# lhn0323/BEVFUSION-3D_object_detection

Hardware: AMD Instinct MI355X
Metric: nuScenes frames/sec (6-cam+LiDAR BEVFusion fwd+bwd) (higher is better)
Workload: dtype bf16; 1 GPU; full: BEVFusion camera+LiDAR (ResNet-50, LSS 6x256x704, hard voxelize 40k pts, sparse encoder, ConvFuser, SECOND/SECONDFPN, TransFusion head + Hungarian targets + focal/L1/gaussian-focal losses) fwd + bwd + clip + AdamW, bf16 autocast, fp32 index paths; global_batch=4, points_per_frame=40000, parallelism=independent frames per rank, execution=eager launches on 2 HIP queues (camera / BEV chain, LiDAR branch), view_transform_conv_dtype=bf16, head_fp32_conv=three bf16 products per multiply, fp32 accumulation (2^-16 relative per product), dense_weight_gradients=one grouped launch per tile shape at the end of the backward pass, backward_pass_thread=caller, trainable_params=37361053

## Files before the change

### bevfusion-3d_object_detection_amd/_lib.py

```python
import ctypes
import os

import torch

_HERE = os.path.dirname(os.path.abspath(__file__))
LIB_PATH = os.path.join(_HERE, "csrc", "libbevfusion_hip.so")

_c_int = ctypes.c_int
_c_vp = ctypes.c_void_p
_c_sz = ctypes.c_size_t

SIGNATURES = {
    "bfhip_abi_version": (_c_int, []),
    "bfhip_last_error": (ctypes.c_char_p, []),
    "bfhip_profile_enable": (None, [_c_int]),
    "bfhip_profile_read": (_c_int, [_c_int, _c_vp, _c_vp, _c_int]),
    "bfhip_bev_pool_fwd": (_c_int, [_c_vp] * 5 + [_c_int] * 7 + [_c_vp, _c_vp]),
    "bfhip_bev_pool_bwd": (_c_int, [_c_vp] * 5 + [_c_int] * 8 + [_c_vp, _c_vp]),
    "bfhip_dynamic_voxelize": (_c_int, [_c_vp, _c_vp, _c_int, _c_int, _c_vp, _c_vp, _c_vp]),
    "bfhip_hard_voxelize_workspace_bytes": (_c_sz, [_c_int, _c_int, _c_int]),
    "bfhip_hard_voxelize": (_c_int, [_c_vp, _c_int, _c_int, _c_vp, _c_vp, _c_vp, _c_vp, _c_vp,
                                     _c_int, _c_int, _c_vp, _c_sz, _c_vp, _c_vp]),
    "bfhip_bev_plan_workspace_bytes": (_c_sz, [ctypes.c_longlong, ctypes.c_longlong]),
    "bfhip_bev_plan": (_c_int, [_c_vp] * 7 + [_c_int] * 4 + [_c_vp] * 3 + [_c_vp] * 11 + [_c_int, _c_vp, _c_sz, _c_vp]),
# ... 22 lines not shown
    "bfhip_sparse_to_bev": (_c_int, [_c_vp, _c_vp] + [_c_int] * 6 + [_c_vp, _c_vp]),
    "bfhip_bev_to_sparse": (_c_int, [_c_vp, _c_vp] + [_c_int] * 6 + [_c_vp, _c_vp]),
    "bfhip_dynamic_scatter_workspace_bytes": (_c_sz, [_c_int]),
    "bfhip_dynamic_scatter_fwd": (_c_int, [_c_vp, _c_vp, _c_int, _c_int, _c_int] + [_c_vp] * 5 + [_c_vp, _c_sz, _c_vp]),
    "bfhip_dynamic_scatter_bwd_workspace_bytes": (_c_sz, [_c_int, _c_int]),
    "bfhip_dynamic_scatter_bwd": (_c_int, [_c_vp] * 6 + [_c_int] * 4 + [_c_vp, _c_sz, _c_vp]),
    "bfhip_voxel_mean": (_c_int, [_c_vp, _c_vp, _c_int, _c_int, _c_int, _c_vp, _c_vp]),
    "bfhip_voxel_compact_mean": (_c_int, [_c_vp] * 4 + [_c_int] * 5 + [_c_vp] * 4),
    "bfhip_depth_lift_bwd_workspace_bytes": (_c_sz, []),
    "bfhip_depth_lift_bwd": (_c_int, [_c_vp, _c_vp, ctypes.c_longlong, _c_vp, _c_vp, _c_sz, _c_vp]),
    "bfhip_rasterise_depth_workspace_bytes": (_c_sz, [_c_int] * 3),
    "bfhip_rasterise_depth": (_c_int, [_c_vp, _c_int, _c_int] + [_c_vp] * 4 + [_c_int] * 3 + [_c_vp, _c_vp] + [_c_int] * 3 +
                              [_c_vp, _c_vp, _c_sz, _c_vp]),
    "bfhip_depth_histogram": (_c_int, [_c_vp] + [_c_int] * 6 + [_c_vp, _c_vp, _c_vp, _c_vp]),
    "bfhip_bn1d_workspace_bytes": (_c_sz, [_c_int, _c_int]),
    "bfhip_bn1d_fwd": (_c_int, [_c_vp] * 4 + [_c_int, _c_int, ctypes.c_float, ctypes.c_float, _c_int] + [_c_vp] * 5 +
                       [_c_vp, _c_sz, _c_vp]),
    "bfhip_bn1d_bwd": (_c_int, [_c_vp] * 5 + [_c_int] * 3 + [_c_vp] * 4 + [_c_vp, _c_sz, _c_vp]),
    "bfhip_sparse_to_bev_nhwc": (_c_int, [_c_vp, _c_vp] + [_c_int] * 7 + [_c_vp, _c_vp]),
    "bfhip_bev_nhwc_to_sparse": (_c_int, [_c_vp, ctypes.c_longlong, ctypes.c_longlong, ctypes.c_longlong, _c_int, _c_vp, _c_int,
                                          _c_int, _c_int, _c_vp, _c_vp]),
    "bfhip_bn2d_supported": (_c_int, [ctypes.c_longlong, _c_int, _c_int]),
    "bfhip_bn2d_workspace_bytes": (_c_sz, [ctypes.c_longlong, _c_int, _c_int]),
    "bfhip_colsum": (_c_int, [_c_vp, ctypes.c_longlong, _c_int, _c_int, _c_vp, _c_vp, _c_sz, _c_vp]),
    "bfhip_bn2d_fwd": (_c_int, [_c_vp] * 4 + [ctypes.c_longlong, _c_int, _c_int, ctypes.c_float, ctypes.c_float, _c_int] +
                       [_c_vp] * 5 + [_c_vp, _c_sz, _c_vp]),
    "bfhip_bn2d_bwd": (_c_int, [_c_vp] * 5 + [ctypes.c_longlong, _c_int, _c_int, _c_int] + [_c_vp] * 4 + [_c_vp, _c_sz, _c_vp]),
    "bfhip_xty_workspace_bytes": (_c_sz, [ctypes.c_longlong, _c_int, _c_int]),
    "bfhip_xty": (_c_int, [_c_vp, _c_vp, ctypes.c_longlong, _c_int, _c_int, _c_int, _c_vp, _c_vp, _c_sz, _c_vp]),
    "bfhip_attn_max_queries": (_c_int, []),
    "bfhip_attn_workspace_bytes": (_c_sz, [_c_int] * 4),
    "bfhip_attn_fwd": (_c_int, [_c_vp] * 3 + [_c_int] * 4 + [ctypes.c_float, ctypes.c_float, ctypes.c_ulonglong, _c_vp, _c_vp,
                                                             _c_vp, _c_vp, _c_sz, _c_vp]),
    "bfhip_attn_bwd": (_c_int, [_c_vp] * 6 + [_c_int] * 4 + [ctypes.c_float, ctypes.c_float, ctypes.c_ulonglong] + [_c_vp] * 4 +
                       [_c_vp, _c_sz, _c_vp]),
    "bfhip_attn_dropout_mask": (_c_int, [_c_int] * 4 + [ctypes.c_float, ctypes.c_ulonglong, _c_vp, _c_vp, _c_vp]),
    "bfhip_upsample2x_nhwc": (_c_int, [_c_vp, _c_vp] + [_c_int] * 6 + [_c_vp]),
    "bfhip_maxpool3x3s2_fwd": (_c_int, [_c_vp] + [_c_int] * 4 + [_c_vp, _c_vp, _c_vp]),
    "bfhip_maxpool3x3s2_bwd": (_c_int, [_c_vp, _c_vp] + [_c_int] * 4 + [_c_vp, _c_vp]),
    "bfhip_circle_nms": (_c_int, [_c_vp, _c_int, ctypes.c_float, _c_int, _c_vp, _c_vp, _c_vp]),
    "bfhip_rotate_nms_workspace_bytes": (_c_sz, [_c_int, _c_int]),
    "bfhip_rotate_nms": (_c_int, [_c_vp, _c_vp, _c_int, ctypes.c_float, _c_int, _c_int, _c_vp, _c_vp, _c_vp, _c_sz, _c_vp]),
    "bfhip_decode_boxes": (_c_int, [_c_vp] * 5 + [_c_int] * 4 + [_c_vp, _c_vp, _c_vp]),
    "bfhip_assign_cost": (_c_int, [_c_vp, _c_int, _c_vp, _c_int, _c_int, _c_int, _c_vp, _c_int, _c_vp, _c_vp] + [_c_int] * 3 +
                          [_c_vp] * 4),
    "bfhip_hungarian": (_c_int, [_c_vp, _c_vp, _c_int, _c_int, _c_int, _c_vp, _c_vp, _c_vp]),
# ... 181 lines not shown
```

### bevfusion-3d_object_detection_amd/csrc/bn2d.hip

```cpp
#include <algorithm>
#include <map>
#include <mutex>

#include "common.h"

namespace bfhip {
namespace {

typedef unsigned short bf16_t;

template <typename T> struct Vec;
template <> struct Vec<float> {
  static constexpr int V = 4;
  static __device__ __forceinline__ void load(const float *p, float *o) {
    float4 v = *(const float4 *)p;
    o[0] = v.x; o[1] = v.y; o[2] = v.z; o[3] = v.w;
  }
  static __device__ __forceinline__ void store(float *p, const float *o) { *(float4 *)p = make_float4(o[0], o[1], o[2], o[3]); }
};
template <> struct Vec<bf16_t> {
  static constexpr int V = 8;
  static __device__ __forceinline__ void load(const bf16_t *p, float *o) {
    uint4 v = *(const uint4 *)p;
    const unsigned w[4] = {v.x, v.y, v.z, v.w};
#pragma unroll
    for (int i = 0; i < 4; ++i) {
      o[2 * i] = __uint_as_float(w[i] << 16);
      o[2 * i + 1] = __uint_as_float(w[i] & 0xffff0000u);
    }
  }
  static __device__ __forceinline__ unsigned rne(float f) {
    unsigned u = __float_as_uint(f);
    if ((u & 0x7fffffffu) > 0x7f800000u) return (u >> 16) | 0x40u;
    return (u + 0x7fffu + ((u >> 16) & 1u)) >> 16;
  }
  static __device__ __forceinline__ void store(bf16_t *p, const float *o) {
    uint4 v;
    v.x = rne(o[0]) | (rne(o[1]) << 16);
    v.y = rne(o[2]) | (rne(o[3]) << 16);
    v.z = rne(o[4]) | (rne(o[5]) << 16);
    v.w = rne(o[6]) | (rne(o[7]) << 16);
    *(uint4 *)p = v;
  }
};
// ... 71 lines not shown
    st_agent(&cnt[1 + g], 0);
    s_flag = __hip_atomic_fetch_add(&cnt[0], 1, __ATOMIC_RELAXED, __HIP_MEMORY_SCOPE_AGENT) == tr.ng - 1;
  }
  __syncthreads();
  if (!s_flag) return;
  if (t == 0) st_agent(&cnt[0], 0);
  if (own) {
    double s = 0.0, s2 = 0.0;
    for (int g2 = 0; g2 < tr.ng; ++g2) {
      s += ld_agent(&tr.gp[((size_t)g2 * 2 + 0) * C + c]);
      s2 += ld_agent(&tr.gp[((size_t)g2 * 2 + 1) * C + c]);
    }
    fin(c, s, s2);
  }
}

struct FwdFin {
  long long M;
  const int *m_dev;
  int C;
  float eps, momentum;
  const float *gamma, *beta;
  float *stats, *running_mean, *running_var;
  __device__ __forceinline__ void operator()(int c, double s, double s2) const {
    long long Mv = M;
    if (m_dev) { long long mv = *m_dev; Mv = mv < 1 ? 1 : (mv < M ? mv : M); }
    double mean = s / (double)Mv;
    double var = s2 / (double)Mv - mean * mean;
    if (var < 0.0) var = 0.0;
    float invstd = (float)(1.0 / sqrt(var + (double)eps));
    float a = gamma[c] * invstd;
    stats[c] = (float)mean;
    stats[C + c] = invstd;
    stats[2 * C + c] = a;
    stats[3 * C + c] = beta[c] - (float)mean * a;
    if (running_mean) {
      double unbiased = Mv > 1 ? var * (double)Mv / (double)(Mv - 1) : var;
      running_mean[c] = (float)((1.0 - momentum) * running_mean[c] + momentum * mean);
      running_var[c] = (float)((1.0 - momentum) * running_var[c] + momentum * unbiased);
    }
  }
};

struct BwdFin {
  long long M;
  const int *m_dev;
  int C;
  const float *stats;
  float *dgb, *coef;
  __device__ __forceinline__ void operator()(int c, double s, double s2) const {
    long long Mv = M;
    if (m_dev) { long long mv = *m_dev; Mv = mv < 1 ? 1 : (mv < M ? mv : M); }
    const float mean = stats[c], invstd = stats[C + c], a = stats[2 * C + c];
    const float dbeta = (float)s, dgamma = (float)(s2 * (double)invstd);
    dgb[c] = dgamma;
    dgb[C + c] = dbeta;
    const float invM = (float)(1.0 / (double)Mv);
    const float c2 = -a * invstd * dgamma * invM;
    coef[c] = a;
    coef[C + c] = c2;
    coef[2 * C + c] = -a * dbeta * invM - c2 * mean;
  }
};

struct SumFin {
  int C;
  float *out;
  __device__ __forceinline__ void operator()(int c, double s, double) const { out[c] = (float)s; }
};

template <typename T>
__global__ __launch_bounds__(256) void bn2d_stats_kernel(const T *__restrict__ x, long long M, int C, Map mp,
                                                         float *__restrict__ partial, Tree tr, FwdFin fin) {
  constexpr int V = Vec<T>::V;
  __shared__ float sm[2 * 256 * V];
  const int t = threadIdx.x, cv = blockIdx.y * mp.Lb + t % mp.Lb, rl = t / mp.Lb;
  const bool live = rl < mp.R && cv * V < C;
  float s0[V], s1[V];
#pragma unroll
  for (int j = 0; j < V; ++j) { s0[j] = 0.f; s1[j] = 0.f; }
  if (live) {
    const long long r0 = (long long)blockIdx.x * mp.rpb, r1 = r0 + mp.rpb < M ? r0 + mp.rpb : M;
    const T *p = x + (size_t)cv * V;
    long long r = r0 + rl;
    for (; r + 3LL * mp.R < r1; r += 4LL * mp.R) {
      float v[4][V];
#pragma unroll
      for (int u = 0; u < 4; ++u) Vec<T>::load(p + (size_t)(r + (long long)u * mp.R) * C, v[u]);
#pragma unroll
      for (int u = 0; u < 4; ++u)
#pragma unroll
        for (int j = 0; j < V; ++j) { s0[j] += v[u][j]; s1[j] += v[u][j] * v[u][j]; }
    }
    for (; r < r1; r += mp.R) {
      float v[V];
      Vec<T>::load(p + (size_t)r * C, v);
#pragma unroll
      for (int j = 0; j < V; ++j) { s0[j] += v[j]; s1[j] += v[j] * v[j]; }
    }
  }
  combine_rows<V>(s0, s1, mp.Lb, mp.R, C, partial, sm);
  finish_in_last_block(partial, tr, C, blockIdx.y * mp.Lb * V, mp.Lb * V, fin);
}

constexpr int kFinLanes = 64, kFinThreads = 8 * kFinLanes;
__device__ __forceinline__ void reduce_partials8(const float *__restrict__ partial, int nblk, int C, int c, bool ok,
                                                 double &s, double &s2) {
  __shared__ double sm[2][kFinThreads];
  const int t = threadIdx.x, kl = t >> 3;
  double a = 0.0, b = 0.0;
  if (ok) {
    for (int k0 = kl; k0 < nblk; k0 += 16 * kFinLanes) {
      float v0[16], v1[16];
#pragma unroll
      for (int u = 0; u < 16; ++u) {
        const int k = k0 + u * kFinLanes, kc = k < nblk ? k : nblk - 1;
        v0[u] = partial[((size_t)kc * 2 + 0) * C + c];
        v1[u] = partial[((size_t)kc * 2 + 1) * C + c];
      }
#pragma unroll
      for (int u = 0; u < 16; ++u)
        if (k0 + u * kFinLanes < nblk) { a += (double)v0[u]; b += (double)v1[u]; }
    }
  }
  sm[0][t] = a;
  sm[1][t] = b;
  __syncthreads();
  double x = 0.0, y = 0.0;
  if (t < 64) {
    const int ch = t & 7, g = t >> 3;
#pragma unroll
    for (int j = 0; j < 8; ++j) { x += sm[0][(g * 8 + j) * 8 + ch]; y += sm[1][(g * 8 + j) * 8 + ch]; }
  }
  __syncthreads();
  if (t < 64) { sm[0][t] = x; sm[1][t] = y; }
  __syncthreads();
  s = 0.0; s2 = 0.0;
  if (t < 8)
#pragma unroll
    for (int g = 0; g < 8; ++g) { s += sm[0][g * 8 + t]; s2 += sm[1][g * 8 + t]; }
}

template <typename Fin>
__global__ __launch_bounds__(kFinThreads) void bn2d_finalize_kernel(const float *__restrict__ partial, int nblk, Fin fin) {
  const int c = blockIdx.x * 8 + (threadIdx.x & 7);
  double s, s2;
  reduce_partials8(partial, nblk, fin.C, c, c < fin.C, s, s2);
  if (threadIdx.x >= 8 || c >= fin.C) return;
  fin(c, s, s2);
}

template <typename T, bool RES, bool RELU>
__global__ __launch_bounds__(256) void bn2d_apply_kernel(const T *__restrict__ x, const T *__restrict__ res,
                                                         const float *__restrict__ stats, long long M, int C, Map mp,
                                                         T *__restrict__ y, unsigned char *__restrict__ relu_mask) {
  constexpr int V = Vec<T>::V;
  const int t = threadIdx.x, cv = blockIdx.y * mp.Lb + t % mp.Lb, rl = t / mp.Lb;
  const bool live = rl < mp.R && cv * V < C;
  if (!live) return;
  float a[V], b[V];
#pragma unroll
  for (int j = 0; j < V; ++j) { a[j] = stats[2 * C + cv * V + j]; b[j] = stats[3 * C + cv * V + j]; }
  const long long r0 = (long long)blockIdx.x * mp.rpb, r1 = r0 + mp.rpb < M ? r0 + mp.rpb : M;
  const size_t col = (size_t)cv * V;
  long long r = r0 + rl;
  for (; r + mp.R < r1; r += 2LL * mp.R) {
    float v[2][V], q[2][V];
#pragma unroll
    for (int u = 0; u < 2; ++u) {
      Vec<T>::load(x + (size_t)(r + (long long)u * mp.R) * C + col, v[u]);
      if (RES) Vec<T>::load(res + (size_t)(r + (long long)u * mp.R) * C + col, q[u]);
    }
// ... 8 lines not shown
        v[u][j] = (RELU && !(o > 0.f)) ? 0.f : o;
      }
      Vec<T>::store(y + (size_t)(r + (long long)u * mp.R) * C + col, v[u]);
      if (V == 8 && relu_mask) relu_mask[(size_t)(r + (long long)u * mp.R) * (C >> 3) + cv] = (unsigned char)bits;
    }
  }
  for (; r < r1; r += mp.R) {
    float v[V], q[V];
    Vec<T>::load(x + (size_t)r * C + col, v);
    if (RES) Vec<T>::load(res + (size_t)r * C + col, q);
    unsigned bits = 0;
#pragma unroll
    for (int j = 0; j < V; ++j) {
      float o = v[j] * a[j] + b[j];
      if (RES) o += q[j];
      if (o > 0.f) bits |= 1u << j;
      v[j] = (RELU && !(o > 0.f)) ? 0.f : o;
    }
    Vec<T>::store(y + (size_t)r * C + col, v);
    if (V == 8 && relu_mask) relu_mask[(size_t)r * (C >> 3) + cv] = (unsigned char)bits;
  }
}

template <typename T, int MASK>
__device__ __forceinline__ void masked_grad(float *g, const float *xv, const float *yv, const float *a, const float *b) {
  constexpr int V = Vec<T>::V;
  const unsigned bits = MASK == 3 ? __float_as_uint(yv[0]) : 0u;
#pragma unroll
  for (int j = 0; j < V; ++j) {
    if (MASK == 1 && !(xv[j] * a[j] + b[j] > 0.f)) g[j] = 0.f;
    if (MASK == 2 && !(yv[j] > 0.f)) g[j] = 0.f;
    if (MASK == 3 && !((bits >> j) & 1u)) g[j] = 0.f;
  }
}

template <typename T, int MASK>
__global__ __launch_bounds__(256) void bn2d_bwd_reduce_kernel(const T *__restrict__ dy, const T *__restrict__ x,
                                                              const T *__restrict__ y,
                                                              const float *__restrict__ stats, long long M, int C,
                                                              Map mp, float *__restrict__ partial, Tree tr, BwdFin fin) {
  constexpr int V = Vec<T>::V;
  __shared__ float sm[2 * 256 * V];
  const int t = threadIdx.x, cv = blockIdx.y * mp.Lb + t % mp.Lb, rl = t / mp.Lb;
  const bool live = rl < mp.R && cv * V < C;
  float s0[V], s1[V];
#pragma unroll
  for (int j = 0; j < V; ++j) { s0[j] = 0.f; s1[j] = 0.f; }
  if (live) {
    float mean[V], a[V], b[V];
#pragma unroll
    for (int j = 0; j < V; ++j) {
      mean[j] = stats[cv * V + j];
      a[j] = stats[2 * C + cv * V + j];
      b[j] = stats[3 * C + cv * V + j];
    }
    const long long r0 = (long long)blockIdx.x * mp.rpb, r1 = r0 + mp.rpb < M ? r0 + mp.rpb : M;
// ... 67 lines not shown
#pragma unroll
    for (int u = 0; u < 2; ++u) {
      size_t off = (size_t)(r + (long long)u * mp.R) * C + col;
      masked_grad<T, MASK>(g[u], xv[u], yv[u], a, b);
      if (DRES) Vec<T>::store(dres + off, g[u]);
#pragma unroll
      for (int j = 0; j < V; ++j) xv[u][j] = c1[j] * g[u][j] + c2[j] * xv[u][j] + c3[j];
      Vec<T>::store(dx + off, xv[u]);
    }
  }
  for (; r < r1; r += mp.R) {
    float g[V], xv[V], yv[V];
    size_t off = (size_t)r * C + col;
    Vec<T>::load(dy + off, g);
    Vec<T>::load(x + off, xv);
    if (MASK == 2) Vec<T>::load(y + off, yv);
    if (MASK == 3) yv[0] = __uint_as_float(((const unsigned char *)y)[(size_t)r * (C >> 3) + cv]);
    masked_grad<T, MASK>(g, xv, yv, a, b);
    if (DRES) Vec<T>::store(dres + off, g);
#pragma unroll
    for (int j = 0; j < V; ++j) xv[j] = c1[j] * g[j] + c2[j] * xv[j] + c3[j];
    Vec<T>::store(dx + off, xv);
  }
}

inline int elem_size(int dtype) { return dtype == 1 ? 2 : 4; }

inline bool shape_ok(long long M, int C, int dtype) {
  const int V = 16 / elem_size(dtype);
  return M > 0 && C >= V && C % V == 0 && C <= 65536;
}

inline Map make_map(long long M, int C, int dtype, dim3 *grid) {
  const int es = elem_size(dtype), V = 16 / es, L = C / V;
  Map mp;
  mp.Lb = L < 32 ? L : 32;
  mp.R = 256 / mp.Lb;
  const int CT = (L + mp.Lb - 1) / mp.Lb;
  long long S = 1024;
  S = std::min(S, (M + 4LL * mp.R - 1) / (4LL * mp.R));
  S = std::min(S, (long long)std::max(1, 2048 / CT));
  S = std::min(S, std::max(1LL, M * es / 128));
  S = std::max(S, 1LL);
  long long rpb = ((M + S - 1) / S + mp.R - 1) / mp.R * mp.R;
  S = (M + rpb - 1) / rpb;
  mp.rpb = (int)rpb;
  *grid = dim3((unsigned)S, (unsigned)CT);
  return mp;
}

template <typename T>
int run_fwd(const void *x, const void *res, const float *stats, long long M, int C, Map mp, dim3 grid, int relu, void *y,
            hipStream_t s, unsigned char *relu_mask = nullptr) {
#define BFHIP_BN2D_APPLY(RES, RELU)                                                                             \
  hipLaunchKernelGGL((bn2d_apply_kernel<T, RES, RELU>), grid, dim3(256), 0, s, (const T *)x, (const T *)res, \
                     stats, M, C, mp, (T *)y, (RES && RELU) ? relu_mask : (unsigned char *)nullptr)
  if (res) { if (relu) BFHIP_BN2D_APPLY(true, true); else BFHIP_BN2D_APPLY(true, false); }
  else { if (relu) BFHIP_BN2D_APPLY(false, true); else BFHIP_BN2D_APPLY(false, false); }
#undef BFHIP_BN2D_APPLY
  return 0;
}

template <typename T, int MASK>
void run_bwd(const void *dy, const void *x, const void *y, const float *stats, long long M, int C, Map mp, dim3 grid,
             float *partial, float *coef, Tree tr, BwdFin fin, void *dx, void *dres, hipStream_t s) {
  hipLaunchKernelGGL((bn2d_bwd_reduce_kernel<T, MASK>), grid, dim3(256), 0, s, (const T *)dy, (const T *)x,
                     (const T *)y, stats, M, C, mp, partial, tr, fin);
  if (!tr.cnt) hipLaunchKernelGGL(bn2d_finalize_kernel<BwdFin>, dim3(ceil_div(C, 8)), dim3(kFinThreads), 0, s, partial, tr.nblk, fin);
  if (dres)
    hipLaunchKernelGGL((bn2d_bwd_apply_kernel<T, MASK, true>), grid, dim3(256), 0, s, (const T *)dy, (const T *)x,
                       (const T *)y, stats, coef, M, C, mp, (T *)dx, (T *)dres);
  else
    hipLaunchKernelGGL((bn2d_bwd_apply_kernel<T, MASK, false>), grid, dim3(256), 0, s, (const T *)dy,
                       (const T *)x, (const T *)y, stats, coef, M, C, mp, (T *)dx, (T *)nullptr);
}

constexpr int kSlabInts = 16384;
constexpr int kSlabs = 32;

inline bool fold_enabled() {
  static const bool on = [] { const char *e = env_str("BFHIP_BN2D_FOLD"); return e && e[0] == '1'; }();
  return on;
}

int *arrival_counters(hipStream_t stream) {
  static std::mutex mu;
  static std::map<int, int *> pool;
  static std::map<std::pair<int, hipStream_t>, int> slot;
  static std::map<int, int> used;
  int dev = 0;
  if (hipGetDevice(&dev) != hipSuccess) return nullptr;
  std::lock_guard<std::mutex> lock(mu);
  auto it = pool.find(dev);
  if (it == pool.end()) {
    int *p = nullptr;
    const size_t bytes = (size_t)kSlabs * kSlabInts * sizeof(int);
    if (hipMalloc((void **)&p, bytes) != hipSuccess || hipMemset(p, 0, bytes) != hipSuccess) {
// ... 25 lines not shown
  pl->ng = (pl->nblk + kGroup - 1) / kGroup;
  size_t off = 0;
  pl->partial = (float *)((char *)workspace + off); off += align_up((size_t)pl->nblk * 2 * C * sizeof(float), 256);
  pl->coef = (float *)((char *)workspace + off); off += align_up((size_t)3 * C * sizeof(float), 256);
  pl->gp = (double *)((char *)workspace + off); off += align_up((size_t)pl->ng * 2 * C * sizeof(double), 256);
  return off;
}

}
}

using namespace bfhip;

BFHIP_EXPORT int bfhip_bn2d_supported(long long M, int C, int dtype) {
  return (dtype == 0 || dtype == 1) && shape_ok(M, C, dtype) ? 1 : 0;
}

BFHIP_EXPORT size_t bfhip_bn2d_workspace_bytes(long long M, int C, int dtype) {
  if (!bfhip_bn2d_supported(M, C, dtype)) return 0;
  Plan pl;
  return plan_bytes(M, C, dtype, &pl, nullptr);
}

BFHIP_EXPORT int bfhip_colsum(const void *x, long long M, int C, int dtype, float *out, void *workspace, size_t workspace_bytes,
                              void *stream_) {
  hipStream_t s = (hipStream_t)stream_;
  BFHIP_REQUIRE(bfhip_bn2d_supported(M, C, dtype), "colsum: unsupported shape M=%lld C=%d dtype=%d", M, C, dtype);
  BFHIP_REQUIRE(x && out && ((uintptr_t)x % 16) == 0, "colsum: null or misaligned pointer");
  if (!workspace || workspace_bytes < bfhip_bn2d_workspace_bytes(M, C, dtype)) { set_error("colsum: workspace too small"); return BFHIP_E_WORKSPACE; }
  Plan pl;
  plan_bytes(M, C, dtype, &pl, workspace);
  Tree tr{nullptr, pl.gp, pl.nblk, pl.ng};
  FwdFin none{};
  if (dtype == 1)
    hipLaunchKernelGGL(bn2d_stats_kernel<bf16_t>, pl.grid, dim3(256), 0, s, (const bf16_t *)x, M, C, pl.mp, pl.partial, tr, none);
  else
    hipLaunchKernelGGL(bn2d_stats_kernel<float>, pl.grid, dim3(256), 0, s, (const float *)x, M, C, pl.mp, pl.partial, tr, none);
  hipLaunchKernelGGL(bn2d_finalize_kernel<SumFin>, dim3(ceil_div(C, 8)), dim3(kFinThreads), 0, s, pl.partial, pl.nblk, SumFin{C, out});
  return check_launch("colsum");
}

BFHIP_EXPORT int bfhip_bn2d_fwd(const void *x, const void *residual, const float *gamma, const float *beta,
                                long long M, int C, int dtype, float eps, float momentum, int relu,
                                float *running_mean, float *running_var, float *stats, void *y, const int32_t *m_dev,
                                void *workspace, size_t workspace_bytes, void *stream_) {
  hipStream_t s = (hipStream_t)stream_;
  BFHIP_REQUIRE(bfhip_bn2d_supported(M, C, dtype), "bn2d_fwd: unsupported shape M=%lld C=%d dtype=%d", M, C, dtype);
  BFHIP_REQUIRE(x && gamma && beta && stats && y, "bn2d_fwd: null pointer");
  BFHIP_REQUIRE(((uintptr_t)x % 16) == 0 && ((uintptr_t)y % 16) == 0 && ((uintptr_t)residual % 16) == 0,
                "bn2d_fwd: tensors must be 16-byte aligned");
  if (!workspace || workspace_bytes < bfhip_bn2d_workspace_bytes(M, C, dtype)) { set_error("bn2d_fwd: workspace too small"); return BFHIP_E_WORKSPACE; }
  Plan pl;
  plan_bytes(M, C, dtype, &pl, workspace);
  int *cnt = fold_enabled() ? arrival_counters(s) : nullptr;
  if (!cnt && fold_enabled()) return BFHIP_E_LAUNCH;
  BFHIP_REQUIRE((long long)pl.grid.y * (1 + pl.ng) <= kSlabInts, "bn2d_fwd: too many column tiles");
  Tree tr{cnt, pl.gp, pl.nblk, pl.ng};
  FwdFin fin{M, m_dev, C, eps, momentum, gamma, beta, stats, running_mean, running_var};
  ProfScope ps;
  prof_begin(BFHIP_OP_BN2D_FWD, s, &ps);
  if (dtype == 1)
    hipLaunchKernelGGL(bn2d_stats_kernel<bf16_t>, pl.grid, dim3(256), 0, s, (const bf16_t *)x, M, C, pl.mp, pl.partial, tr, fin);
  else
    hipLaunchKernelGGL(bn2d_stats_kernel<float>, pl.grid, dim3(256), 0, s, (const float *)x, M, C, pl.mp, pl.partial, tr, fin);
  if (!cnt) hipLaunchKernelGGL(bn2d_finalize_kernel<FwdFin>, dim3(ceil_div(C, 8)), dim3(kFinThreads), 0, s, pl.partial, pl.nblk, fin);
  if (dtype == 1) run_fwd<bf16_t>(x, residual, stats, M, C, pl.mp, pl.grid, relu, y, s);
  else run_fwd<float>(x, residual, stats, M, C, pl.mp, pl.grid, relu, y, s);
  prof_end(&ps);
  return check_launch("bn2d_fwd");
}

static int bn2d_fwd_partials_impl(const void *x, const void *residual, const float *gamma, const float *beta, long long M, int C,
                                  int dtype, float eps, float momentum, int relu, float *running_mean, float *running_var,
                                  float *stats, void *y, const float *partial, int nblk, const int32_t *m_dev,
                                  unsigned char *relu_mask, void *stream_) {
  hipStream_t s = (hipStream_t)stream_;
  BFHIP_REQUIRE(!relu_mask || (dtype == 1 && relu && residual), "bn2d_fwd_partials: a ReLU bit mask needs bf16 + residual + ReLU");
  BFHIP_REQUIRE(bfhip_bn2d_supported(M, C, dtype), "bn2d_fwd_partials: unsupported shape M=%lld C=%d dtype=%d", M, C, dtype);
  BFHIP_REQUIRE(x && gamma && beta && stats && y && partial && nblk > 0, "bn2d_fwd_partials: null pointer");
  BFHIP_REQUIRE(((uintptr_t)x % 16) == 0 && ((uintptr_t)y % 16) == 0 && ((uintptr_t)residual % 16) == 0,
                "bn2d_fwd_partials: tensors must be 16-byte aligned");
  dim3 grid;
  Map mp = make_map(M, C, dtype, &grid);
  FwdFin fin{M, m_dev, C, eps, momentum, gamma, beta, stats, running_mean, running_var};
  ProfScope ps;
  prof_begin(BFHIP_OP_BN2D_FWD, s, &ps);
  hipLaunchKernelGGL(bn2d_finalize_kernel<FwdFin>, dim3(ceil_div(C, 8)), dim3(kFinThreads), 0, s, partial, nblk, fin);
  if (dtype == 1) run_fwd<bf16_t>(x, residual, stats, M, C, mp, grid, relu, y, s, relu_mask);
  else run_fwd<float>(x, residual, stats, M, C, mp, grid, relu, y, s);
  prof_end(&ps);
  return check_launch("bn2d_fwd_partials");
}

BFHIP_EXPORT int bfhip_bn2d_fwd_partials(const void *x, const void *residual, const float *gamma, const float *beta,
                                         long long M, int C, int dtype, float eps, float momentum, int relu,
                                         float *running_mean, float *running_var, float *stats, void *y,
                                         const float *partial, int nblk, const int32_t *m_dev, void *stream_) {
  return bn2d_fwd_partials_impl(x, residual, gamma, beta, M, C, dtype, eps, momentum, relu, running_mean, running_var, stats, y,
                                partial, nblk, m_dev, nullptr, stream_);
}

BFHIP_EXPORT int bfhip_bn2d_fwd_partials_mask(const void *x, const void *residual, const float *gamma, const float *beta,
                                              long long M, int C, int dtype, float eps, float momentum, int relu,
                                              float *running_mean, float *running_var, float *stats, void *y,
                                              const float *partial, int nblk, const int32_t *m_dev, unsigned char *relu_mask,
                                              void *stream_) {
  BFHIP_REQUIRE(relu_mask, "bn2d_fwd_partials_mask: null mask");
  return bn2d_fwd_partials_impl(x, residual, gamma, beta, M, C, dtype, eps, momentum, relu, running_mean, running_var, stats, y,
                                partial, nblk, m_dev, relu_mask, stream_);
}

static int bn2d_bwd_impl(const void *dy, const void *x, const void *y, const unsigned char *relu_mask, const float *stats,
                         const float *gamma, long long M, int C, int dtype, int relu, void *dx, void *dres, float *dgb,
                         const int32_t *m_dev, void *workspace, size_t workspace_bytes, void *stream_) {
  hipStream_t s = (hipStream_t)stream_;
  BFHIP_REQUIRE(!relu_mask || (dtype == 1 && relu), "bn2d_bwd: a ReLU bit mask needs bf16 + ReLU");
  if (relu_mask) y = relu_mask;
  BFHIP_REQUIRE(bfhip_bn2d_supported(M, C, dtype), "bn2d_bwd: unsupported shape M=%lld C=%d dtype=%d", M, C, dtype);
  BFHIP_REQUIRE(dy && x && stats && gamma && dx && dgb, "bn2d_bwd: null pointer");
  BFHIP_REQUIRE(((uintptr_t)dy % 16) == 0 && ((uintptr_t)x % 16) == 0 && ((uintptr_t)dx % 16) == 0 &&
                    ((uintptr_t)y % 16) == 0 && ((uintptr_t)dres % 16) == 0, "bn2d_bwd: tensors must be 16-byte aligned");
  if (!workspace || workspace_bytes < bfhip_bn2d_workspace_bytes(M, C, dtype)) { set_error("bn2d_bwd: workspace too small"); return BFHIP_E_WORKSPACE; }
  Plan pl;
  plan_bytes(M, C, dtype, &pl, workspace);
  int *cnt = fold_enabled() ? arrival_counters(s) : nullptr;
  if (!cnt && fold_enabled()) return BFHIP_E_LAUNCH;
  BFHIP_REQUIRE((long long)pl.grid.y * (1 + pl.ng) <= kSlabInts, "bn2d_bwd: too many column tiles");
  Tree tr{cnt, pl.gp, pl.nblk, pl.ng};
  BwdFin fin{M, m_dev, C, stats, dgb, pl.coef};
  const int mask = !relu ? 0 : (relu_mask ? 3 : (y ? 2 : 1));
  ProfScope ps;
  prof_begin(BFHIP_OP_BN2D_BWD, s, &ps);
#define BFHIP_BN2D_BWD(T, MASK) run_bwd<T, MASK>(dy, x, y, stats, M, C, pl.mp, pl.grid, pl.partial, pl.coef, tr, fin, dx, dres, s)
  if (dtype == 1) {
    if (mask == 0) BFHIP_BN2D_BWD(bf16_t, 0);
    else if (mask == 1) BFHIP_BN2D_BWD(bf16_t, 1);
    else if (mask == 3) BFHIP_BN2D_BWD(bf16_t, 3);
    else BFHIP_BN2D_BWD(bf16_t, 2);
  } else {
    if (mask == 0) BFHIP_BN2D_BWD(float, 0);
    else if (mask == 1) BFHIP_BN2D_BWD(float, 1);
    else BFHIP_BN2D_BWD(float, 2);
  }
#undef BFHIP_BN2D_BWD
  prof_end(&ps);
  return check_launch("bn2d_bwd");
}

BFHIP_EXPORT int bfhip_bn2d_bwd(const void *dy, const void *x, const void *y, const float *stats, const float *gamma,
                                long long M, int C, int dtype, int relu, void *dx, void *dres, float *dgb,
                                const int32_t *m_dev, void *workspace, size_t workspace_bytes, void *stream_) {
  return bn2d_bwd_impl(dy, x, y, nullptr, stats, gamma, M, C, dtype, relu, dx, dres, dgb, m_dev, workspace, workspace_bytes, stream_);
}

BFHIP_EXPORT int bfhip_bn2d_bwd_mask(const void *dy, const void *x, const unsigned char *relu_mask, const float *stats,
                                     const float *gamma, long long M, int C, int dtype, void *dx, void *dres, float *dgb,
// ... 6 lines not shown
```

### include/bevfusion_hip.h

```cpp
#ifndef BEVFUSION_HIP_H_
#define BEVFUSION_HIP_H_

#include <stddef.h>
#include <stdint.h>

#ifdef __cplusplus
extern "C" {
#endif

#define BFHIP_OK 0
#define BFHIP_E_INVALID (-1)
#define BFHIP_E_WORKSPACE (-2)
#define BFHIP_E_LAUNCH (-3)

#define BFHIP_REDUCE_SUM 0
#define BFHIP_REDUCE_MEAN 1
#define BFHIP_REDUCE_MAX 2

#define BFHIP_OP_BEV_POOL_FWD 0
#define BFHIP_OP_BEV_POOL_BWD 1
#define BFHIP_OP_HARD_VOXELIZE 2
#define BFHIP_OP_DYNAMIC_VOXELIZE 3
#define BFHIP_OP_LIFT_SPLAT_FWD 4
#define BFHIP_OP_LIFT_SPLAT_BWD 5
// ... 125 lines not shown
                             int dtype, const int32_t *indices, int N, int C, int Z, float *grad_feats, void *stream);

size_t bfhip_depth_lift_bwd_workspace_bytes(void);
int bfhip_depth_lift_bwd(const void *dy, const void *d, long long M, float *out, void *workspace, size_t workspace_bytes, void *stream);
size_t bfhip_rasterise_depth_workspace_bytes(int ncam, int iH, int iW);
int bfhip_rasterise_depth(const float *points, int n, int f, const float *inv_rot, const float *aug_trans,
                          const float *lidar2image, const float *img_aug, int ncam, int iH, int iW,
                          float *depth, float *counts, int fH, int fW, int D, const float *dbound_host,
                          void *workspace, size_t workspace_bytes, void *stream);
int bfhip_depth_histogram(const float *depth, int BN, int iH, int iW, int fH, int fW, int D,
                          const float *dbound_host, float *counts, float *distr, void *stream);

size_t bfhip_bn1d_workspace_bytes(int N, int C);
int bfhip_bn1d_fwd(const float *x, const float *residual, const float *gamma, const float *beta, int N, int C,
                   float eps, float momentum, int relu, float *running_mean, float *running_var, float *stats,
                   float *y, const int32_t *n_rows_dev, void *workspace, size_t workspace_bytes, void *stream);
int bfhip_bn1d_bwd(const float *dy, const float *y, const float *x, const float *stats, const float *gamma, int N,
                   int C, int relu, float *dx, float *dres, float *dgb, const int32_t *n_rows_dev, void *workspace,
                   size_t workspace_bytes, void *stream);

int bfhip_bn2d_supported(long long M, int C, int dtype);
int bfhip_colsum(const void *x, long long M, int C, int dtype, float *out, void *workspace, size_t workspace_bytes, void *stream);
size_t bfhip_bn2d_workspace_bytes(long long M, int C, int dtype);
int bfhip_bn2d_fwd(const void *x, const void *residual, const float *gamma, const float *beta, long long M, int C,
                   int dtype, float eps, float momentum, int relu, float *running_mean, float *running_var,
                   float *stats, void *y, const int32_t *m_dev, void *workspace, size_t workspace_bytes, void *stream);
int bfhip_bn2d_bwd(const void *dy, const void *x, const void *y, const float *stats, const float *gamma, long long M,
                   int C, int dtype, int relu, void *dx, void *dres, float *dgb, const int32_t *m_dev, void *workspace,
                   size_t workspace_bytes, void *stream);

size_t bfhip_xty_workspace_bytes(long long K, int M, int N);
int bfhip_xty(const void *X, const void *Y, long long K, int M, int N, int dtype, float *out, void *workspace,
              size_t workspace_bytes, void *stream);

int bfhip_attn_max_queries(void);
size_t bfhip_attn_workspace_bytes(int B, int H, int Lq, int Lk);
int bfhip_attn_fwd(const void *Q, const void *K, const void *V, int B, int H, int Lq, int Lk, float scale,
                   float dropout_p, unsigned long long seed, const unsigned long long *seed_dev, void *O, float *lse,
                   void *workspace, size_t workspace_bytes, void *stream);
int bfhip_attn_bwd(const void *Q, const void *K, const void *V, const void *O, const void *dO, const float *lse, int B,
                   int H, int Lq, int Lk, float scale, float dropout_p, unsigned long long seed,
                   const unsigned long long *seed_dev, void *dQ, void *dK, void *dV, void *workspace, size_t workspace_bytes,
                   void *stream);
int bfhip_attn_dropout_mask(int B, int H, int Lq, int Lk, float dropout_p, unsigned long long seed,
                            const unsigned long long *seed_dev, unsigned char *mask, void *stream);

// ... 207 lines not shown
```

Baseline: 155.6 frames/s.

## Add row-per-thread BN2d apply kernels and deeper-prefetch finalize reduction

Adds a streaming plan that, for small shapes (few pieces), launches new one-row-per-thread apply kernels for BN2d forward and backward. These load the raw vectors up front and use a flat grid instead of the looping multi-row blocks. The finalize kernel gains a DEEP variant that preloads per-channel parameters before the reduction and uses a shorter unrolled sweep when there are few partial blocks. The aim is lower latency for the many small BN launches, at the cost of more kernel variants and launching more blocks for mid-size shapes. It is gated by the BFHIP_BN2D_GEOM environment variable, which is on by default, and also exports a plan query function.

```diff
diff --git a/bevfusion-3d_object_detection_amd/_lib.py b/bevfusion-3d_object_detection_amd/_lib.py
--- a/bevfusion-3d_object_detection_amd/_lib.py
+++ b/bevfusion-3d_object_detection_amd/_lib.py
@@ -68,6 +68,7 @@
                                           _c_int, _c_int, _c_vp, _c_vp]),
     "bfhip_bn2d_supported": (_c_int, [ctypes.c_longlong, _c_int, _c_int]),
     "bfhip_bn2d_workspace_bytes": (_c_sz, [ctypes.c_longlong, _c_int, _c_int]),
+    "bfhip_bn2d_plan": (_c_int, [ctypes.c_longlong, _c_int, _c_int, _c_vp]),
     "bfhip_colsum": (_c_int, [_c_vp, ctypes.c_longlong, _c_int, _c_int, _c_vp, _c_vp, _c_sz, _c_vp]),
     "bfhip_bn2d_fwd": (_c_int, [_c_vp] * 4 + [ctypes.c_longlong, _c_int, _c_int, ctypes.c_float, ctypes.c_float, _c_int] +
                        [_c_vp] * 5 + [_c_vp, _c_sz, _c_vp]),
diff --git a/bevfusion-3d_object_detection_amd/csrc/bn2d.hip b/bevfusion-3d_object_detection_amd/csrc/bn2d.hip
--- a/bevfusion-3d_object_detection_amd/csrc/bn2d.hip
+++ b/bevfusion-3d_object_detection_amd/csrc/bn2d.hip
@@ -12,6 +12,9 @@
 template <typename T> struct Vec;
 template <> struct Vec<float> {
   static constexpr int V = 4;
+  typedef float4 Raw;
+  static __device__ __forceinline__ Raw ldraw(const float *p) { return *(const float4 *)p; }
+  static __device__ __forceinline__ void unpack(const Raw &v, float *o) { o[0] = v.x; o[1] = v.y; o[2] = v.z; o[3] = v.w; }
   static __device__ __forceinline__ void load(const float *p, float *o) {
     float4 v = *(const float4 *)p;
     o[0] = v.x; o[1] = v.y; o[2] = v.z; o[3] = v.w;
@@ -20,6 +23,16 @@
 };
 template <> struct Vec<bf16_t> {
   static constexpr int V = 8;
+  typedef uint4 Raw;
+  static __device__ __forceinline__ Raw ldraw(const bf16_t *p) { return *(const uint4 *)p; }
+  static __device__ __forceinline__ void unpack(const Raw &v, float *o) {
+    const unsigned w[4] = {v.x, v.y, v.z, v.w};
+#pragma unroll
+    for (int i = 0; i < 4; ++i) {
+      o[2 * i] = __uint_as_float(w[i] << 16);
+      o[2 * i + 1] = __uint_as_float(w[i] & 0xffff0000u);
+    }
+  }
   static __device__ __forceinline__ void load(const bf16_t *p, float *o) {
     uint4 v = *(const uint4 *)p;
     const unsigned w[4] = {v.x, v.y, v.z, v.w};
@@ -137,22 +150,33 @@
   float eps, momentum;
   const float *gamma, *beta;
   float *stats, *running_mean, *running_var;
-  __device__ __forceinline__ void operator()(int c, double s, double s2) const {
-    long long Mv = M;
-    if (m_dev) { long long mv = *m_dev; Mv = mv < 1 ? 1 : (mv < M ? mv : M); }
+  struct Pre { long long Mv; float gamma, beta, rmean, rvar; };
+  __device__ __forceinline__ Pre preload(int c) const {
+    Pre p;
+    p.Mv = M;
+    if (m_dev) { long long mv = *m_dev; p.Mv = mv < 1 ? 1 : (mv < M ? mv : M); }
+    p.gamma = gamma[c];
+    p.beta = beta[c];
+    p.rmean = running_mean ? running_mean[c] : 0.f;
+    p.rvar = running_mean ? running_var[c] : 0.f;
+    return p;
+  }
+  __device__ __forceinline__ void operator()(int c, double s, double s2) const { (*this)(c, s, s2, preload(c)); }
+  __device__ __forceinline__ void operator()(int c, double s, double s2, const Pre &p) const {
+    const long long Mv = p.Mv;
     double mean = s / (double)Mv;
     double var = s2 / (double)Mv - mean * mean;
     if (var < 0.0) var = 0.0;
     float invstd = (float)(1.0 / sqrt(var + (double)eps));
-    float a = gamma[c] * invstd;
+    float a = p.gamma * invstd;
     stats[c] = (float)mean;
     stats[C + c] = invstd;
     stats[2 * C + c] = a;
-    stats[3 * C + c] = beta[c] - (float)mean * a;
+    stats[3 * C + c] = p.beta - (float)mean * a;
     if (running_mean) {
       double unbiased = Mv > 1 ? var * (double)Mv / (double)(Mv - 1) : var;
-      running_mean[c] = (float)((1.0 - momentum) * running_mean[c] + momentum * mean);
-      running_var[c] = (float)((1.0 - momentum) * running_var[c] + momentum * unbiased);
+      running_mean[c] = (float)((1.0 - momentum) * p.rmean + momentum * mean);
+      running_var[c] = (float)((1.0 - momentum) * p.rvar + momentum * unbiased);
     }
   }
 };
@@ -163,10 +187,20 @@
   int C;
   const float *stats;
   float *dgb, *coef;
-  __device__ __forceinline__ void operator()(int c, double s, double s2) const {
-    long long Mv = M;
-    if (m_dev) { long long mv = *m_dev; Mv = mv < 1 ? 1 : (mv < M ? mv : M); }
-    const float mean = stats[c], invstd = stats[C + c], a = stats[2 * C + c];
+  struct Pre { long long Mv; float mean, invstd, a; };
+  __device__ __forceinline__ Pre preload(int c) const {
+    Pre p;
+    p.Mv = M;
+    if (m_dev) { long long mv = *m_dev; p.Mv = mv < 1 ? 1 : (mv < M ? mv : M); }
+    p.mean = stats[c];
+    p.invstd = stats[C + c];
+    p.a = stats[2 * C + c];
+    return p;
+  }
+  __device__ __forceinline__ void operator()(int c, double s, double s2) const { (*this)(c, s, s2, preload(c)); }
+  __device__ __forceinline__ void operator()(int c, double s, double s2, const Pre &p) const {
+    const long long Mv = p.Mv;
+    const float mean = p.mean, invstd = p.invstd, a = p.a;
     const float dbeta = (float)s, dgamma = (float)(s2 * (double)invstd);
     dgb[c] = dgamma;
     dgb[C + c] = dbeta;
@@ -181,7 +215,10 @@
 struct SumFin {
   int C;
   float *out;
+  struct Pre {};
+  __device__ __forceinline__ Pre preload(int) const { return Pre{}; }
   __device__ __forceinline__ void operator()(int c, double s, double) const { out[c] = (float)s; }
+  __device__ __forceinline__ void operator()(int c, double s, double, const Pre &) const { out[c] = (float)s; }
 };
 
 template <typename T>
@@ -219,12 +256,33 @@
 }
 
 constexpr int kFinLanes = 64, kFinThreads = 8 * kFinLanes;
+
+template <int U>
+__device__ __forceinline__ void sweep_partials(const float *__restrict__ partial, int nblk, int C, int c, int k0, double &a,
+                                               double &b) {
+  float v0[U], v1[U];
+#pragma unroll
+  for (int u = 0; u < U; ++u) {
+    const int k = k0 + u * kFinLanes, kc = k < nblk ? k : nblk - 1;
+    v0[u] = partial[((size_t)kc * 2 + 0) * C + c];
+    v1[u] = partial[((size_t)kc * 2 + 1) * C + c];
+  }
+#pragma unroll
+  for (int u = 0; u < U; ++u)
+    if (k0 + u * kFinLanes < nblk) { a += (double)v0[u]; b += (double)v1[u]; }
+}
+
+template <bool DEEP>
 __device__ __forceinline__ void reduce_partials8(const float *__restrict__ partial, int nblk, int C, int c, bool ok,
                                                  double &s, double &s2) {
   __shared__ double sm[2][kFinThreads];
   const int t = threadIdx.x, kl = t >> 3;
   double a = 0.0, b = 0.0;
-  if (ok) {
+  if (ok && DEEP) {
+    if (nblk <= 4 * kFinLanes) sweep_partials<4>(partial, nblk, C, c, kl, a, b);
+    else
+      for (int k0 = kl; k0 < nblk; k0 += 16 * kFinLanes) sweep_partials<16>(partial, nblk, C, c, k0, a, b);
+  } else if (ok) {
     for (int k0 = kl; k0 < nblk; k0 += 16 * kFinLanes) {
       float v0[16], v1[16];
 #pragma unroll
@@ -256,13 +314,23 @@
     for (int g = 0; g < 8; ++g) { s += sm[0][g * 8 + t]; s2 += sm[1][g * 8 + t]; }
 }
 
-template <typename Fin>
+template <typename Fin, bool DEEP>
 __global__ __launch_bounds__(kFinThreads) void bn2d_finalize_kernel(const float *__restrict__ partial, int nblk, Fin fin) {
   const int c = blockIdx.x * 8 + (threadIdx.x & 7);
+  const bool lead = threadIdx.x < 8 && c < fin.C;
+  typename Fin::Pre pre{};
+  if (DEEP && lead) pre = fin.preload(c);
   double s, s2;
-  reduce_partials8(partial, nblk, fin.C, c, c < fin.C, s, s2);
-  if (threadIdx.x >= 8 || c >= fin.C) return;
-  fin(c, s, s2);
+  reduce_partials8<DEEP>(partial, nblk, fin.C, c, c < fin.C, s, s2);
+  if (!lead) return;
+  if (DEEP) fin(c, s, s2, pre);
+  else fin(c, s, s2);
+}
+
+template <typename Fin>
+void launch_finalize(bool deep, int C, hipStream_t s, const float *partial, int nblk, Fin fin) {
+  if (deep) hipLaunchKernelGGL((bn2d_finalize_kernel<Fin, true>), dim3(ceil_div(C, 8)), dim3(kFinThreads), 0, s, partial, nblk, fin);
+  else hipLaunchKernelGGL((bn2d_finalize_kernel<Fin, false>), dim3(ceil_div(C, 8)), dim3(kFinThreads), 0, s, partial, nblk, fin);
 }
 
 template <typename T, bool RES, bool RELU>
@@ -317,6 +385,33 @@
   }
 }
 
+template <typename T, bool RES, bool RELU>
+__global__ __launch_bounds__(256) void bn2d_apply_row_kernel(const T *__restrict__ x, const T *__restrict__ res,
+                                                             const float *__restrict__ stats, long long M, int C, Map mp,
+                                                             T *__restrict__ y, unsigned char *__restrict__ relu_mask) {
+  constexpr int V = Vec<T>::V;
+  const int t = threadIdx.x, cv = blockIdx.y * mp.Lb + t % mp.Lb, rl = t / mp.Lb;
+  const long long r = (long long)blockIdx.x * mp.rpb + rl;
+  if (!(rl < mp.R && cv * V < C && r < M)) return;
+  const size_t off = (size_t)r * C + (size_t)cv * V;
+  const typename Vec<T>::Raw xr = Vec<T>::ldraw(x + off), qr = RES ? Vec<T>::ldraw(res + off) : xr;
+  float a[V], b[V], v[V], q[V];
+#pragma unroll
+  for (int j = 0; j < V; ++j) { a[j] = stats[2 * C + cv * V + j]; b[j] = stats[3 * C + cv * V + j]; }
+  Vec<T>::unpack(xr, v);
+  Vec<T>::unpack(qr, q);
+  unsigned bits = 0;
+#pragma unroll
+  for (int j = 0; j < V; ++j) {
+    float o = v[j] * a[j] + b[j];
+    if (RES) o += q[j];
+    if (o > 0.f) bits |= 1u << j;
+    v[j] = (RELU && !(o > 0.f)) ? 0.f : o;
+  }
+  Vec<T>::store(y + off, v);
+  if (V == 8 && relu_mask) relu_mask[(size_t)r * (C >> 3) + cv] = (unsigned char)bits;
+}
+
 template <typename T, int MASK>
 __device__ __forceinline__ void masked_grad(float *g, const float *xv, const float *yv, const float *a, const float *b) {
   constexpr int V = Vec<T>::V;
@@ -327,6 +422,31 @@
     if (MASK == 2 && !(yv[j] > 0.f)) g[j] = 0.f;
     if (MASK == 3 && !((bits >> j) & 1u)) g[j] = 0.f;
   }
+}
+
+template <typename T, int MASK> struct BwdRow {
+  typename Vec<T>::Raw g, x, y;
+  unsigned bits;
+};
+template <typename T, int MASK>
+__device__ __forceinline__ BwdRow<T, MASK> load_bwd_row(const T *__restrict__ dy, const T *__restrict__ x, const T *__restrict__ y,
+                                                        long long r, int C, size_t col, int cv) {
+  BwdRow<T, MASK> w;
+  const size_t off = (size_t)r * C + col;
+  w.g = Vec<T>::ldraw(dy + off);
+  w.x = Vec<T>::ldraw(x + off);
+  if (MASK == 2) w.y = Vec<T>::ldraw(y + off);
+  if (MASK == 3) w.bits = ((const unsigned char *)y)[(size_t)r * (C >> 3) + cv];
+  return w;
+}
+template <typename T, int MASK>
+__device__ __forceinline__ void unpack_bwd_row(const BwdRow<T, MASK> &w, float *g, float *xv, const float *a, const float *b) {
+  float yv[Vec<T>::V];
+  Vec<T>::unpack(w.g, g);
+  Vec<T>::unpack(w.x, xv);
+  if (MASK == 2) Vec<T>::unpack(w.y, yv);
+  if (MASK == 3) yv[0] = __uint_as_float(w.bits);
+  masked_grad<T, MASK>(g, xv, yv, a, b);
 }
 
 template <typename T, int MASK>
@@ -440,6 +560,33 @@
     for (int j = 0; j < V; ++j) xv[j] = c1[j] * g[j] + c2[j] * xv[j] + c3[j];
     Vec<T>::store(dx + off, xv);
   }
+}
+
+template <typename T, int MASK, bool DRES>
+__global__ __launch_bounds__(256) void bn2d_bwd_apply_row_kernel(const T *__restrict__ dy, const T *__restrict__ x,
+                                                                 const T *__restrict__ y, const float *__restrict__ stats,
+                                                                 const float *__restrict__ coef, long long M, int C, Map mp,
+                                                                 T *__restrict__ dx, T *__restrict__ dres) {
+  constexpr int V = Vec<T>::V;
+  const int t = threadIdx.x, cv = blockIdx.y * mp.Lb + t % mp.Lb, rl = t / mp.Lb;
+  const long long r = (long long)blockIdx.x * mp.rpb + rl;
+  if (!(rl < mp.R && cv * V < C && r < M)) return;
+  const size_t off = (size_t)r * C + (size_t)cv * V;
+  const BwdRow<T, MASK> w = load_bwd_row<T, MASK>(dy, x, y, r, C, (size_t)cv * V, cv);
+  float a[V], b[V], c1[V], c2[V], c3[V], g[V], xv[V];
+#pragma unroll
+  for (int j = 0; j < V; ++j) {
+    a[j] = stats[2 * C + cv * V + j];
+    b[j] = stats[3 * C + cv * V + j];
+    c1[j] = coef[cv * V + j];
+    c2[j] = coef[C + cv * V + j];
+    c3[j] = coef[2 * C + cv * V + j];
+  }
+  unpack_bwd_row<T, MASK>(w, g, xv, a, b);
+  if (DRES) Vec<T>::store(dres + off, g);
+#pragma unroll
+  for (int j = 0; j < V; ++j) xv[j] = c1[j] * g[j] + c2[j] * xv[j] + c3[j];
+  Vec<T>::store(dx + off, xv);
 }
 
 inline int elem_size(int dtype) { return dtype == 1 ? 2 : 4; }
@@ -467,30 +614,66 @@
   return mp;
 }
 
+inline bool geom_enabled() {
+  static const bool on = [] { const char *e = env_str("BFHIP_BN2D_GEOM"); return !(e && e[0] == '0'); }();
+  return on;
+}
+
+constexpr int kStreamPiecesFwd = 2304, kStreamPiecesBwd = 1536;
+struct StreamPlan {
+  Map mp;
+  dim3 grid;
+  bool row;
+};
+inline StreamPlan make_stream_plan(long long M, int C, int dtype, bool bwd) {
+  StreamPlan sp;
+  sp.mp = make_map(M, C, dtype, &sp.grid);
+  const long long pieces = (M + sp.mp.R - 1) / sp.mp.R * sp.grid.y;
+  sp.row = geom_enabled() && pieces <= (bwd ? kStreamPiecesBwd : kStreamPiecesFwd);
+  if (sp.row) {
+    sp.mp.rpb = sp.mp.R;
+    sp.grid.x = (unsigned)((M + sp.mp.R - 1) / sp.mp.R);
+  }
+  return sp;
+}
+
 template <typename T>
-int run_fwd(const void *x, const void *res, const float *stats, long long M, int C, Map mp, dim3 grid, int relu, void *y,
+int run_fwd(const void *x, const void *res, const float *stats, long long M, int C, const StreamPlan &sp, int relu, void *y,
             hipStream_t s, unsigned char *relu_mask = nullptr) {
-#define BFHIP_BN2D_APPLY(RES, RELU)                                                                             \
-  hipLaunchKernelGGL((bn2d_apply_kernel<T, RES, RELU>), grid, dim3(256), 0, s, (const T *)x, (const T *)res, \
-                     stats, M, C, mp, (T *)y, (RES && RELU) ? relu_mask : (unsigned char *)nullptr)
+#define BFHIP_BN2D_APPLY_K(KERNEL, RES, RELU)                                                         \
+  hipLaunchKernelGGL(KERNEL, sp.grid, dim3(256), 0, s, (const T *)x, (const T *)res, stats, M, C, sp.mp, (T *)y, \
+                     (RES && RELU) ? relu_mask : (unsigned char *)nullptr)
+#define BFHIP_BN2D_APPLY(RES, RELU)                                                            \
+  do {                                                                                         \
+    if (sp.row) BFHIP_BN2D_APPLY_K((bn2d_apply_row_kernel<T, RES, RELU>), RES, RELU);          \
+    else BFHIP_BN2D_APPLY_K((bn2d_apply_kernel<T, RES, RELU>), RES, RELU);                     \
+  } while (0)
   if (res) { if (relu) BFHIP_BN2D_APPLY(true, true); else BFHIP_BN2D_APPLY(true, false); }
   else { if (relu) BFHIP_BN2D_APPLY(false, true); else BFHIP_BN2D_APPLY(false, false); }
 #undef BFHIP_BN2D_APPLY
+#undef BFHIP_BN2D_APPLY_K
   return 0;
+}
+
+template <typename T, int MASK, bool DRES>
+void run_bwd_apply(const void *dy, const void *x, const void *y, const float *stats, const float *coef, long long M, int C,
+                   const StreamPlan &sp, void *dx, void *dres, hipStream_t s) {
+#define BFHIP_BN2D_BWD_APPLY(KERNEL)                                                                                    \
+  hipLaunchKernelGGL(KERNEL, sp.grid, dim3(256), 0, s, (const T *)dy, (const T *)x, (const T *)y, stats, coef, M, C, sp.mp, \
+                     (T *)dx, (T *)dres)
+  if (sp.row) BFHIP_BN2D_BWD_APPLY((bn2d_bwd_apply_row_kernel<T, MASK, DRES>));
+  else BFHIP_BN2D_BWD_APPLY((bn2d_bwd_apply_kernel<T, MASK, DRES>));
+#undef BFHIP_BN2D_BWD_APPLY
 }
 
 template <typename T, int MASK>
 void run_bwd(const void *dy, const void *x, const void *y, const float *stats, long long M, int C, Map mp, dim3 grid,
-             float *partial, float *coef, Tree tr, BwdFin fin, void *dx, void *dres, hipStream_t s) {
+             const StreamPlan &sp, float *partial, float *coef, Tree tr, BwdFin fin, void *dx, void *dres, hipStream_t s) {
   hipLaunchKernelGGL((bn2d_bwd_reduce_kernel<T, MASK>), grid, dim3(256), 0, s, (const T *)dy, (const T *)x,
                      (const T *)y, stats, M, C, mp, partial, tr, fin);
-  if (!tr.cnt) hipLaunchKernelGGL(bn2d_finalize_kernel<BwdFin>, dim3(ceil_div(C, 8)), dim3(kFinThreads), 0, s, partial, tr.nblk, fin);
-  if (dres)
-    hipLaunchKernelGGL((bn2d_bwd_apply_kernel<T, MASK, true>), grid, dim3(256), 0, s, (const T *)dy, (const T *)x,
-                       (const T *)y, stats, coef, M, C, mp, (T *)dx, (T *)dres);
-  else
-    hipLaunchKernelGGL((bn2d_bwd_apply_kernel<T, MASK, false>), grid, dim3(256), 0, s, (const T *)dy,
-                       (const T *)x, (const T *)y, stats, coef, M, C, mp, (T *)dx, (T *)nullptr);
+  if (!tr.cnt) launch_finalize(geom_enabled(), C, s, partial, tr.nblk, fin);
+  if (dres) run_bwd_apply<T, MASK, true>(dy, x, y, stats, coef, M, C, sp, dx, dres, s);
+  else run_bwd_apply<T, MASK, false>(dy, x, y, stats, coef, M, C, sp, dx, nullptr, s);
 }
 
 constexpr int kSlabInts = 16384;
@@ -562,6 +745,21 @@
   return plan_bytes(M, C, dtype, &pl, nullptr);
 }
 
+BFHIP_EXPORT int bfhip_bn2d_plan(long long M, int C, int dtype, int *out_host) {
+  BFHIP_REQUIRE(out_host, "bn2d_plan: bad arguments");
+  BFHIP_REQUIRE(bfhip_bn2d_supported(M, C, dtype), "bn2d_plan: unsupported shape M=%lld C=%d dtype=%d", M, C, dtype);
+  dim3 grid;
+  const Map mp = make_map(M, C, dtype, &grid);
+  const int red[8] = {mp.Lb, mp.R, mp.rpb, (int)grid.x, (int)grid.y, mp.rpb / mp.R, 4, 2};
+  for (int i = 0; i < 8; ++i) out_host[i] = red[i];
+  for (int bwd = 0; bwd < 2; ++bwd) {
+    const StreamPlan sp = make_stream_plan(M, C, dtype, bwd != 0);
+    const int str[8] = {sp.mp.Lb, sp.mp.R, sp.mp.rpb, (int)sp.grid.x, (int)sp.grid.y, sp.mp.rpb / sp.mp.R, sp.row ? 1 : 2, sp.row ? 1 : 0};
+    for (int i = 0; i < 8; ++i) out_host[8 + 8 * bwd + i] = str[i];
+  }
+  return BFHIP_OK;
+}
+
 BFHIP_EXPORT int bfhip_colsum(const void *x, long long M, int C, int dtype, float *out, void *workspace, size_t workspace_bytes,
                               void *stream_) {
   hipStream_t s = (hipStream_t)stream_;
@@ -576,7 +774,7 @@
     hipLaunchKernelGGL(bn2d_stats_kernel<bf16_t>, pl.grid, dim3(256), 0, s, (const bf16_t *)x, M, C, pl.mp, pl.partial, tr, none);
   else
     hipLaunchKernelGGL(bn2d_stats_kernel<float>, pl.grid, dim3(256), 0, s, (const float *)x, M, C, pl.mp, pl.partial, tr, none);
-  hipLaunchKernelGGL(bn2d_finalize_kernel<SumFin>, dim3(ceil_div(C, 8)), dim3(kFinThreads), 0, s, pl.partial, pl.nblk, SumFin{C, out});
+  launch_finalize(geom_enabled(), C, s, pl.partial, pl.nblk, SumFin{C, out});
   return check_launch("colsum");
 }
 
@@ -603,9 +801,10 @@
     hipLaunchKernelGGL(bn2d_stats_kernel<bf16_t>, pl.grid, dim3(256), 0, s, (const bf16_t *)x, M, C, pl.mp, pl.partial, tr, fin);
   else
     hipLaunchKernelGGL(bn2d_stats_kernel<float>, pl.grid, dim3(256), 0, s, (const float *)x, M, C, pl.mp, pl.partial, tr, fin);
-  if (!cnt) hipLaunchKernelGGL(bn2d_finalize_kernel<FwdFin>, dim3(ceil_div(C, 8)), dim3(kFinThreads), 0, s, pl.partial, pl.nblk, fin);
-  if (dtype == 1) run_fwd<bf16_t>(x, residual, stats, M, C, pl.mp, pl.grid, relu, y, s);
-  else run_fwd<float>(x, residual, stats, M, C, pl.mp, pl.grid, relu, y, s);
+  if (!cnt) launch_finalize(geom_enabled(), C, s, pl.partial, pl.nblk, fin);
+  const StreamPlan sp = make_stream_plan(M, C, dtype, false);
+  if (dtype == 1) run_fwd<bf16_t>(x, residual, stats, M, C, sp, relu, y, s);
+  else run_fwd<float>(x, residual, stats, M, C, sp, relu, y, s);
   prof_end(&ps);
   return check_launch("bn2d_fwd");
 }
@@ -620,14 +819,13 @@
   BFHIP_REQUIRE(x && gamma && beta && stats && y && partial && nblk > 0, "bn2d_fwd_partials: null pointer");
   BFHIP_REQUIRE(((uintptr_t)x % 16) == 0 && ((uintptr_t)y % 16) == 0 && ((uintptr_t)residual % 16) == 0,
                 "bn2d_fwd_partials: tensors must be 16-byte aligned");
-  dim3 grid;
-  Map mp = make_map(M, C, dtype, &grid);
+  const StreamPlan sp = make_stream_plan(M, C, dtype, false);
   FwdFin fin{M, m_dev, C, eps, momentum, gamma, beta, stats, running_mean, running_var};
   ProfScope ps;
   prof_begin(BFHIP_OP_BN2D_FWD, s, &ps);
-  hipLaunchKernelGGL(bn2d_finalize_kernel<FwdFin>, dim3(ceil_div(C, 8)), dim3(kFinThreads), 0, s, partial, nblk, fin);
-  if (dtype == 1) run_fwd<bf16_t>(x, residual, stats, M, C, mp, grid, relu, y, s, relu_mask);
-  else run_fwd<float>(x, residual, stats, M, C, mp, grid, relu, y, s);
+  launch_finalize(geom_enabled(), C, s, partial, nblk, fin);
+  if (dtype == 1) run_fwd<bf16_t>(x, residual, stats, M, C, sp, relu, y, s, relu_mask);
+  else run_fwd<float>(x, residual, stats, M, C, sp, relu, y, s);
   prof_end(&ps);
   return check_launch("bn2d_fwd_partials");
 }
@@ -671,7 +869,8 @@
   const int mask = !relu ? 0 : (relu_mask ? 3 : (y ? 2 : 1));
   ProfScope ps;
   prof_begin(BFHIP_OP_BN2D_BWD, s, &ps);
-#define BFHIP_BN2D_BWD(T, MASK) run_bwd<T, MASK>(dy, x, y, stats, M, C, pl.mp, pl.grid, pl.partial, pl.coef, tr, fin, dx, dres, s)
+  const StreamPlan sp = make_stream_plan(M, C, dtype, true);
+#define BFHIP_BN2D_BWD(T, MASK) run_bwd<T, MASK>(dy, x, y, stats, M, C, pl.mp, pl.grid, sp, pl.partial, pl.coef, tr, fin, dx, dres, s)
   if (dtype == 1) {
     if (mask == 0) BFHIP_BN2D_BWD(bf16_t, 0);
     else if (mask == 1) BFHIP_BN2D_BWD(bf16_t, 1);
diff --git a/include/bevfusion_hip.h b/include/bevfusion_hip.h
--- a/include/bevfusion_hip.h
+++ b/include/bevfusion_hip.h
@@ -171,6 +171,7 @@
 int bfhip_bn2d_supported(long long M, int C, int dtype);
 int bfhip_colsum(const void *x, long long M, int C, int dtype, float *out, void *workspace, size_t workspace_bytes, void *stream);
 size_t bfhip_bn2d_workspace_bytes(long long M, int C, int dtype);
+int bfhip_bn2d_plan(long long M, int C, int dtype, int *out_host);
 int bfhip_bn2d_fwd(const void *x, const void *residual, const float *gamma, const float *beta, long long M, int C,
                    int dtype, float eps, float momentum, int relu, float *running_mean, float *running_var,
                    float *stats, void *y, const int32_t *m_dev, void *workspace, size_t workspace_bytes, void *stream);
```

New measurement: 156.7 frames/s, median of 6. Within noise of the previous version (+0.7%).
